# chymaera96/NeuralSampleID

Measured on AMD Instinct MI355X. Metric: audio clips/sec (contrastive step, grafp encoder), higher is better.
Workload: dtype bf16

## Files before the change

neuralsampleid_amd/build.py:

```python
import os
import subprocess
import sys
from concurrent.futures import ThreadPoolExecutor

PKG = os.path.dirname(os.path.abspath(__file__))
CSRC = os.path.join(PKG, "csrc")
ROOT = os.path.dirname(PKG)
LIB = os.path.join(PKG, "libnsid_hip.so")
OBJ_DIR = os.path.join(PKG, "csrc", "_obj")
SOURCES = ["tuning.hip", "gemm.hip", "gemm256.hip", "wsgemm.hip", "ffn_fused.hip", "ffn256_fused.hip", "mrconv_fused.hip", "wgrad.hip", "bn.hip", "knn.hip", "mr.hip", "ntxent.hip", "misc.hip"]
HIPCC = os.environ.get("HIPCC", "/opt/rocm/bin/hipcc")
FLAGS = ["-O3", "--offload-arch=gfx950", "-fPIC", "-std=c++17", "-Wall", "-Wno-unused-function",
         "-fno-gpu-rdc", "-I", os.path.join(ROOT, "include")]


def _newer(a, b):
    return not os.path.exists(b) or os.path.getmtime(a) > os.path.getmtime(b)


def _deps():
    hdrs = [os.path.join(CSRC, "nsid_common.h"), os.path.join(ROOT, "include", "nsid.h")]
    return max(os.path.getmtime(h) for h in hdrs)


def _check_flags() -> None:
    if "-DNSID_" in HIPCC or any(f.startswith("-DNSID_") for f in FLAGS):
        raise RuntimeError("refusing to build the product library with a -DNSID_* switch: use tools/build_variant.sh for diagnosis builds")


def _source_hash() -> str:
    import hashlib
    _check_flags()
    h = hashlib.sha256((HIPCC + " " + " ".join(f for f in FLAGS if f != os.path.join(ROOT, "include"))).encode())
    for f in [os.path.join(CSRC, s) for s in SOURCES] + [os.path.join(CSRC, "nsid_common.h"),
                                                         os.path.join(ROOT, "include", "nsid.h")]:
        h.update(open(f, "rb").read())
    return h.hexdigest()


def build_lib(force: bool = False, verbose: bool = True) -> str:
    stamp = LIB + ".srchash"
    digest = _source_hash()
    if not force and os.path.exists(LIB) and os.path.exists(stamp) and open(stamp).read().strip() == digest:
        return LIB
    force = True
    os.makedirs(OBJ_DIR, exist_ok=True)
    hdr_time = _deps()
    jobs = []
    for src in SOURCES:
        s = os.path.join(CSRC, src)
        o = os.path.join(OBJ_DIR, src.replace(".hip", ".o"))
        if force or _newer(s, o) or os.path.getmtime(o) < hdr_time:
            jobs.append((s, o))

    def compile_one(job):
        s, o = job
        cmd = [HIPCC, *FLAGS, "-c", s, "-o", o]
        r = subprocess.run(cmd, capture_output=True, text=True)
        if r.returncode != 0:
            raise RuntimeError(f"hipcc failed for {s}:\n{r.stderr}")
        if verbose and r.stderr.strip():
            print(r.stderr, file=sys.stderr)
        return o

    if jobs:
        with ThreadPoolExecutor(max_workers=min(6, len(jobs))) as ex:
            list(ex.map(compile_one, jobs))
    objs = [os.path.join(OBJ_DIR, s.replace(".hip", ".o")) for s in SOURCES]
    if jobs or not os.path.exists(LIB):
        r = subprocess.run([HIPCC, "--offload-arch=gfx950", "-shared", "-fPIC", "-o", LIB, *objs],
                           capture_output=True, text=True)
        if r.returncode != 0:
            raise RuntimeError("link failed:\n" + r.stderr)
        if verbose:
            print(f"built {LIB} ({os.path.getsize(LIB) / 1024:.0f} KB)")
    with open(stamp, "w") as f:
        f.write(digest)
    return LIB


if __name__ == "__main__":
    build_lib(force="--force" in sys.argv)
```

neuralsampleid_amd/csrc/gemm.hip:

```cpp
#include <algorithm>
#include <cstdlib>
#include "nsid_common.h"

namespace {

inline float act_slope(int act) { return act == NSID_ACT_RELU ? 0.f : (act == NSID_ACT_LEAKY ? 0.2f : 1.f); }

struct GemmArgs {
  const void* A; long lda; long a_goff;
  const void* B; long ldb; long b_goff;
  void* C; long ldc; long c_goff;
  int I, J, R;
  const float* a_scale; const float* a_shift; float a_slope; long a_aff_goff;
  const float* b_scale; const float* b_shift; float b_slope; long b_aff_goff;
  const float* bias; long bias_goff;
  const void* addend; long ldadd;
  float* stat; long stat_plane;
  long stat_ld;
  int rsplit;
  int rchunk;
  int atomic_out;
  int split_major;
  const void* bn_r; long bn_ldr;
  const float* bn_scale; const float* bn_shift; const float* bn_mean; const float* bn_invstd; float bn_slope;
// ... 934 lines not shown
  p.rchunk = (M + p.rsplit - 1) / p.rsplit;
  return launch_pad<64, 64, false, false, 2>(p, 1, static_cast<hipStream_t>(stream), act_dtype, false);
}

extern "C" int nsid_downsample3_bwd_data(const void* dout, const void* wp, const void* w_odd, int w_dtype, void* dx, int B,
                                         int N, int C, int Cout, int act_dtype, void* stream) {
  NSID_REQUIRE(dout && wp && w_odd && dx && B > 0 && N > 0 && N % 2 == 0 && C > 0 && Cout > 0 && NSID_DTYPE_OK(act_dtype));
  const int ch = act_dtype == NSID_BF16 ? 8 : 4;
  NSID_REQUIRE(C % ch == 0 && Cout % ch == 0 && nsid_aligned16(dout) && nsid_aligned16(wp) && nsid_aligned16(w_odd) &&
               nsid_aligned16(dx) && NSID_DTYPE_OK(w_dtype) && (w_dtype == NSID_F32 || act_dtype == NSID_BF16));
  const int No = N / 2, M = B * No;
  const long esz = act_dtype == NSID_BF16 ? 2 : 4, wsz = w_dtype == NSID_BF16 ? 2 : 4;
  hipStream_t s = static_cast<hipStream_t>(stream);
  const bool wb = w_dtype == NSID_BF16;
  GemmArgs p{};
  p.A = dout; p.lda = Cout; p.a_goff = Cout;
  p.B = static_cast<const char*>(wp) + (long)C * wsz; p.ldb = 3L * C; p.b_goff = 0;
  p.C = dx; p.ldc = 2L * C; p.c_goff = C;
  p.I = M; p.J = C; p.R = Cout;
  p.rsplit = 1; p.rchunk = Cout;
  p.bn_slope = 1.f;
  int rc = C <= 64 ? launch<128, 64, true, false>(p, 1, s, act_dtype, wb) : launch<128, 128, true, false>(p, 1, s, act_dtype, wb);
  if (rc != NSID_OK) return rc;
  GemmArgs q{};
  q.A = dout; q.lda = Cout; q.a_goff = 2L * Cout;
  q.B = w_odd; q.ldb = C; q.b_goff = 0;
  q.C = static_cast<char*>(dx) + (long)C * esz; q.ldc = 2L * C; q.c_goff = C;
  q.I = M; q.J = C; q.R = 2 * Cout;
  q.rsplit = 1; q.rchunk = 2 * Cout;
  q.bn_slope = 1.f;
  q.pad_period = No; q.pad_phase = No - 1; q.pad_c0 = Cout; q.pad_c1 = 2 * Cout; q.pad_safe = 0;
  return C <= 64 ? launch_pad<128, 64, true, false, 1>(q, 1, s, act_dtype, wb)
                 : launch_pad<128, 128, true, false, 1>(q, 1, s, act_dtype, wb);
}

void* g_gemm_trace_host = nullptr;
extern "C" int nsid_debug_gemm_trace(void* buf) {
  g_gemm_trace_host = buf;
  return hipMemcpyToSymbol(HIP_SYMBOL(g_gemm_trace), &buf, sizeof(buf)) == hipSuccess ? NSID_OK : NSID_EINVAL;
}
extern "C" int nsid_set_gemm_precision(int mode) {
  if (mode != NSID_GEMM_FP32 && mode != NSID_GEMM_BF16) return NSID_EINVAL;
  g_gemm_precision = mode;
  return NSID_OK;
}
extern "C" int nsid_get_gemm_precision(void) { return g_gemm_precision; }
extern "C" long nsid_gemm_g256_launches(void) { return g_g256_launches; }
extern "C" int nsid_row_tiles(int M) { return (M + NSID_ROW_TILE - 1) / NSID_ROW_TILE; }

static int linear_fwd_impl(const void* x, int ldx, const void* w, int w_dtype, const float* bias, void* out, int ldo,
                           int M, int Nout, int K, int groups, const float* in_scale, const float* in_shift, int act_in,
                           int act_out, float* stat, int ksplit, int act_dtype, const void* addend, int ldadd,
                           void* stream);

extern "C" int nsid_linear_fwd(const void* x, int ldx, const void* w, int w_dtype, const float* bias, void* out, int ldo,
                               int M, int Nout, int K, int groups, const float* in_scale, const float* in_shift,
                               int act_in, int act_out, float* stat, int ksplit, int act_dtype, void* stream) {
  return linear_fwd_impl(x, ldx, w, w_dtype, bias, out, ldo, M, Nout, K, groups, in_scale, in_shift, act_in, act_out, stat,
                         ksplit, act_dtype, nullptr, 0, stream);
}

extern "C" int nsid_linear_fwd_res(const void* x, int ldx, const void* w, int w_dtype, const float* bias,
                                   const void* addend, int ldadd, void* out, int ldo, int M, int Nout, int K, int groups,
                                   const float* in_scale, const float* in_shift, int act_in, int act_dtype,
                                   void* stream) {
  const int ch = act_dtype == NSID_BF16 ? 8 : 4;
  NSID_REQUIRE(addend && ldadd % ch == 0 && ldadd >= groups * Nout && nsid_aligned16(addend));
  return linear_fwd_impl(x, ldx, w, w_dtype, bias, out, ldo, M, Nout, K, groups, in_scale, in_shift, act_in,
                         NSID_ACT_NONE, nullptr, 1, act_dtype, addend, ldadd, stream);
}

static int linear_fwd_impl(const void* x, int ldx, const void* w, int w_dtype, const float* bias, void* out, int ldo,
                           int M, int Nout, int K, int groups, const float* in_scale, const float* in_shift, int act_in,
                           int act_out, float* stat, int ksplit, int act_dtype, const void* addend, int ldadd,
                           void* stream) {
  NSID_REQUIRE(x && w && out && M > 0 && Nout > 0 && K > 0 && groups > 0 && ksplit >= 1 && NSID_DTYPE_OK(act_dtype));
  NSID_REQUIRE(NSID_DTYPE_OK(w_dtype) && (w_dtype == NSID_F32 || (act_dtype == NSID_BF16 && K % 8 == 0)));
  const int ch = act_dtype == NSID_BF16 ? 8 : 4;
  NSID_REQUIRE(K % ch == 0 && ldx % ch == 0 && nsid_aligned16(x) && nsid_aligned16(w) && K % 4 == 0);
  NSID_REQUIRE(act_dtype == NSID_F32 || (ksplit == 1 && (act_out == NSID_ACT_NONE || act_out == NSID_ACT_RELU) && Nout % 8 == 0 && ldo % 8 == 0));
  NSID_REQUIRE(act_out != NSID_ACT_RELU || (ksplit == 1 && stat == nullptr && addend == nullptr));
  NSID_REQUIRE((ldx >= groups * K || (groups == 1 && ldx > 0)) && ldo >= groups * Nout);
  NSID_REQUIRE(Nout % 4 == 0 && ldo % 4 == 0 && nsid_aligned16(out) && (bias == nullptr || nsid_aligned16(bias)));
  NSID_REQUIRE((in_scale == nullptr) == (in_shift == nullptr));
  NSID_REQUIRE(ksplit == 1 || (stat == nullptr && (act_out == NSID_ACT_NONE || (act_out == NSID_ACT_ELU && act_dtype == NSID_F32))));
  NSID_REQUIRE(act_in != NSID_ACT_ELU && (act_out == NSID_ACT_NONE || act_out == NSID_ACT_ELU || act_out == NSID_ACT_RELU));
  NSID_REQUIRE(in_scale != nullptr || act_in == NSID_ACT_NONE ||
               (act_in == NSID_ACT_RELU && act_dtype == NSID_BF16 && w_dtype == NSID_BF16));
  GemmArgs p{};
  p.A = x; p.lda = ldx; p.a_goff = K;
  p.B = w; p.ldb = K; p.b_goff = (long)Nout * K;
  p.C = out; p.ldc = ldo; p.c_goff = Nout;
  p.I = M; p.J = Nout; p.R = K;
  p.a_scale = in_scale; p.a_shift = in_shift; p.a_slope = act_slope(act_in); p.a_aff_goff = K;
  p.bias = bias; p.bias_goff = Nout;
  p.addend = addend; p.ldadd = ldadd;
  p.stat = stat; p.stat_ld = (long)groups * Nout; p.stat_plane = (long)nsid_row_tiles(M) * groups * Nout;
  p.rsplit = ksplit;
  p.rchunk = (K + ksplit - 1) / ksplit;
  p.atomic_out = ksplit > 1;
  p.relu_out = act_out == NSID_ACT_RELU;
  hipStream_t s = static_cast<hipStream_t>(stream);
  const long t128 = (long)nsid_row_tiles(M) * ((Nout + 127) / 128) * groups;
  const bool half = g_gemm_precision == NSID_GEMM_BF16 || act_dtype == NSID_BF16;
  const int force_narrow = (int)nsid_tune(NSID_T_fwd_narrow);
  bool narrow = half ? (Nout <= 64 || (Nout <= 128 && K <= 256 && in_scale == nullptr)) : Nout <= 64;
  if (half && t128 < 128) narrow = true;
  if (force_narrow >= 0 && Nout > 64) narrow = force_narrow != 0;
  const bool wb = w_dtype == NSID_BF16;
  if ((nsid_tune(NSID_T_ws_gemm) & 1) && act_dtype == NSID_BF16 && wb && ksplit == 1 && act_out == NSID_ACT_NONE && addend == nullptr &&
      act_in != NSID_ACT_ELU) {
    const int rcw = nsid_ws_fwd_launch(x, ldx, w, bias, out, ldo, M, Nout, K, groups, in_scale, in_shift, act_slope(act_in), stat,
                                       p.stat_plane, p.stat_ld, s);
    if (rcw != 1) { nsid_count(NSID_C_ws_fwd); return rcw; }
  }
  const long g256_min = nsid_tune(NSID_T_g256_min);
  if (g256_min > 0 && (stat == nullptr || nsid_tune(NSID_T_g256_train) != 0) && act_dtype == NSID_BF16 && wb && groups == 1 && in_scale == nullptr && ksplit == 1 &&
      (act_out == NSID_ACT_NONE || act_out == NSID_ACT_RELU) && act_in == NSID_ACT_NONE && ldx >= K &&
      (long)(M / 256) * (Nout / 256) >= g256_min) {
    const int rc256 = nsid_gemm256_fwd_launch(x, ldx, w, bias, addend, ldadd, out, ldo, M, Nout, K, act_out == NSID_ACT_RELU, stat,
                                              p.stat_plane, p.stat_ld, s);
    if (rc256 != 1) { ++g_g256_launches; nsid_count(NSID_C_gemm256); return rc256; }
  }
  const int rc = narrow ? launch<128, 64, true, true>(p, groups, s, act_dtype, wb) : launch<128, 128, true, true>(p, groups, s, act_dtype, wb);
  if (rc != NSID_OK || act_out != NSID_ACT_ELU) return rc;
  const long n = (long)M * groups * Nout;
  NSID_LAUNCH(elu_inplace_kernel, dim3((int)((n + 255) / 256 > 2048 ? 2048 : (n + 255) / 256)), dim3(256), 0, s,
              static_cast<float*>(out), (long)M, groups * Nout, (long)ldo);
  return nsid_launch_status();
}

struct AbnArgs {
  const void* r; const float* coef4; int act; void* dr;
};
static int linear_bwd_data_impl(const void* dout, int ldd, const void* w, int w_dtype, const void* addend, int ldadd,
                                void* din, int ldi, int M, int Nout, int K, int groups, int act_dtype, void* stream,
                                const void* bn_r, const float* bn_scale, const float* bn_shift, const float* bn_mean,
                                const float* bn_invstd, int bn_act, float* bn_partial, const AbnArgs* abn = nullptr);

extern "C" int nsid_linear_bwd_data(const void* dout, int ldd, const void* w, int w_dtype, const void* addend, int ldadd,
                                    void* din, int ldi, int M, int Nout, int K, int groups, int act_dtype,
                                    void* stream) {
  return linear_bwd_data_impl(dout, ldd, w, w_dtype, addend, ldadd, din, ldi, M, Nout, K, groups, act_dtype, stream,
                              nullptr, nullptr, nullptr, nullptr, nullptr, NSID_ACT_NONE, nullptr);
}

extern "C" int nsid_linear_bwd_data_bn(const void* dout, int ldd, const void* w, int w_dtype, const void* addend,
                                       int ldadd, void* din, int ldi, int M, int Nout, int K, int groups, int act_dtype,
                                       const void* bn_r, const float* bn_scale, const float* bn_shift,
                                       const float* bn_mean, const float* bn_invstd, int bn_act, float* bn_partial,
                                       void* stream) {
  NSID_REQUIRE(bn_r && bn_scale && bn_shift && bn_mean && bn_invstd && bn_partial && act_dtype == NSID_BF16);
  NSID_REQUIRE(ldi == groups * K && (groups * K) % 8 == 0 && nsid_aligned16(bn_r));
  NSID_REQUIRE(bn_act == NSID_ACT_NONE || bn_act == NSID_ACT_RELU || bn_act == NSID_ACT_LEAKY);
  return linear_bwd_data_impl(dout, ldd, w, w_dtype, addend, ldadd, din, ldi, M, Nout, K, groups, act_dtype, stream,
                              bn_r, bn_scale, bn_shift, bn_mean, bn_invstd, bn_act, bn_partial);
}

extern "C" int nsid_linear_bwd_data_bnapply(const void* dy, const void* r, const float* coef4, int act, void* dr, const void* w,
                                            int w_dtype, const void* addend, int ldadd, void* din, int ldi, int M, int Nout, int K,
                                            int groups, int act_dtype, const void* bn_r, const float* bn_scale,
                                            const float* bn_shift, const float* bn_mean, const float* bn_invstd, int bn_act,
                                            float* bn_partial, void* stream) {
  NSID_REQUIRE(dy && r && coef4 && dr && nsid_aligned16(r) && nsid_aligned16(dr) && nsid_aligned16(coef4));
  NSID_REQUIRE(dr != dy && dr != r);
  NSID_REQUIRE(act == NSID_ACT_NONE || act == NSID_ACT_RELU || act == NSID_ACT_LEAKY);
  if (act_dtype != NSID_BF16 || w_dtype != NSID_BF16 || (groups * Nout) % 8 != 0) return 1;
  if (bn_r != nullptr) {
    NSID_REQUIRE(bn_scale && bn_shift && bn_mean && bn_invstd && bn_partial && ldi == groups * K && (groups * K) % 8 == 0 &&
                 nsid_aligned16(bn_r));
    NSID_REQUIRE(bn_act == NSID_ACT_NONE || bn_act == NSID_ACT_RELU || bn_act == NSID_ACT_LEAKY);
  }
  const AbnArgs abn{r, coef4, act, dr};
  return linear_bwd_data_impl(dy, groups * Nout, w, w_dtype, addend, ldadd, din, ldi, M, Nout, K, groups, act_dtype, stream, bn_r,
                              bn_scale, bn_shift, bn_mean, bn_invstd, bn_act, bn_partial, &abn);
}

static int linear_bwd_data_impl(const void* dout, int ldd, const void* w, int w_dtype, const void* addend, int ldadd,
                                void* din, int ldi, int M, int Nout, int K, int groups, int act_dtype, void* stream,
                                const void* bn_r, const float* bn_scale, const float* bn_shift, const float* bn_mean,
                                const float* bn_invstd, int bn_act, float* bn_partial, const AbnArgs* abn) {
  NSID_REQUIRE(dout && w && din && M > 0 && Nout > 0 && K > 0 && groups > 0 && NSID_DTYPE_OK(act_dtype));
  NSID_REQUIRE(NSID_DTYPE_OK(w_dtype) && (w_dtype == NSID_F32 || (act_dtype == NSID_BF16 && K % 8 == 0)));
  const bool wb = w_dtype == NSID_BF16;
  const int ch = act_dtype == NSID_BF16 ? 8 : 4;
  NSID_REQUIRE(Nout % ch == 0 && K % ch == 0 && ldd % ch == 0 && ldi % ch == 0 && nsid_aligned16(dout) && nsid_aligned16(w));
  NSID_REQUIRE(addend == nullptr || ldadd % ch == 0);
  NSID_REQUIRE(ldd >= groups * Nout && ldi >= groups * K && ldi % 4 == 0 && nsid_aligned16(din));
  NSID_REQUIRE(addend == nullptr || (ldadd % 4 == 0 && ldadd >= groups * K && nsid_aligned16(addend)));
  GemmArgs p{};
  p.A = dout; p.lda = ldd; p.a_goff = Nout;
  p.B = w; p.ldb = K; p.b_goff = (long)Nout * K;
  p.C = din; p.ldc = ldi; p.c_goff = K;
  p.I = M; p.J = K; p.R = Nout;
  p.addend = addend; p.ldadd = ldadd;
  p.rsplit = 1; p.rchunk = Nout;
  p.bn_r = bn_r; p.bn_ldr = (long)groups * K;
  p.bn_scale = bn_scale; p.bn_shift = bn_shift; p.bn_mean = bn_mean; p.bn_invstd = bn_invstd;
  p.bn_slope = act_slope(bn_act);
  p.bn_partial = bn_partial; p.bn_ld = (long)groups * K; p.bn_plane = (long)nsid_row_tiles(M) * groups * K;
  hipStream_t s = static_cast<hipStream_t>(stream);
  const long t128 = (long)nsid_row_tiles(M) * ((K + 127) / 128) * groups;
  const bool half = g_gemm_precision == NSID_GEMM_BF16 || act_dtype == NSID_BF16;
  const int force_narrow = (int)nsid_tune(NSID_T_bwd_narrow);
  bool narrow = half ? (K <= 64 || (K <= 128 && Nout <= 256)) : K <= 64;
  if (half && t128 < 128) narrow = true;
  if (force_narrow >= 0 && K > 64) narrow = force_narrow != 0;
  if ((nsid_tune(NSID_T_ws_gemm) & (abn ? 4 : 2)) && act_dtype == NSID_BF16 && wb &&
      (bn_r == nullptr || bn_partial != nullptr)) {
    const int rcw = nsid_ws_bwd_data_launch(dout, ldd, w, addend, ldadd, din, ldi, M, Nout, K, groups, bn_r, p.bn_ldr, bn_scale, bn_shift,
                                            bn_mean, bn_invstd, p.bn_slope, bn_partial, p.bn_plane, p.bn_ld, abn ? abn->r : nullptr,
                                            abn ? abn->coef4 : nullptr, (long)groups * Nout, abn ? act_slope(abn->act) : 1.f,
                                            abn ? abn->dr : nullptr, (long)groups * Nout, s);
    if (rcw != 1) { nsid_count(abn ? NSID_C_ws_bwd_bnapply : NSID_C_ws_bwd_data); return rcw; }
  }
  if (abn != nullptr) {
    narrow = K <= 64;
    p.abn_r = abn->r; p.abn_coef = abn->coef4; p.abn_plane = (long)groups * Nout; p.abn_slope = act_slope(abn->act);
    p.abn_dr = abn->dr; p.abn_lddr = (long)groups * Nout;
    if (K % (narrow ? 64 : 128) != 0 || M % 128 != 0 || Nout % 64 != 0) return 1;
  }
  if (act_dtype == NSID_F32 && addend == nullptr && bn_r == nullptr && abn == nullptr && groups == 1 && Nout >= 1024 && ldi == K) {
    const long tiles = (long)nsid_row_tiles(M) * ((K + (narrow ? 63 : 127)) / (narrow ? 64 : 128));
    const long maxt = nsid_tune(NSID_T_bwd_split_max_tiles);
    const long S = maxt > 0 && tiles <= maxt ? std::min<long>(256 / tiles, Nout / 256) : 1;
    if (S > 1) {
      const int rcz = nsid_fill_zero(din, (size_t)M * K * 4, stream);
      if (rcz != NSID_OK) return rcz;
      p.rsplit = (int)S;
      p.rchunk = (int)((Nout + S - 1) / S);
      p.atomic_out = 1;
      nsid_count(NSID_C_gemm_bwd_split);
    }
  }
  if (narrow) return launch<128, 64, true, false>(p, groups, s, act_dtype, wb);
  return launch<128, 128, true, false>(p, groups, s, act_dtype, wb);
}

extern "C" int nsid_linear_bwd_weight(const void* dout, int ldd, const void* x, int ldx, float* dw, int M, int Nout,
                                      int K, int groups, const float* in_scale, const float* in_shift, int act_in,
                                      int act_dtype, void* stream) {
  NSID_REQUIRE(dout && x && dw && M > 0 && Nout > 0 && K > 0 && groups > 0 && NSID_DTYPE_OK(act_dtype));
  const int ch = act_dtype == NSID_BF16 ? 8 : 4;
  NSID_REQUIRE(Nout % ch == 0 && K % ch == 0 && ldd % ch == 0 && ldx % ch == 0 && nsid_aligned16(dout) && nsid_aligned16(x));
  NSID_REQUIRE((in_scale == nullptr) == (in_shift == nullptr));
  GemmArgs p{};
  p.A = dout; p.lda = ldd; p.a_goff = Nout;
  p.B = x; p.ldb = ldx; p.b_goff = K;
  p.C = dw; p.ldc = K; p.c_goff = (long)Nout * K;
  p.I = Nout; p.J = K; p.R = M;
  p.b_scale = in_scale; p.b_shift = in_shift; p.b_slope = act_slope(act_in); p.b_aff_goff = K;
  p.atomic_out = 1;
  const bool use_wide = nsid_tune(NSID_T_wgrad_wide) != 0;
  if (use_wide && act_dtype == NSID_BF16 && nsid_aligned16(dout) && nsid_aligned16(x) &&
      (in_scale == nullptr || (nsid_aligned16(in_scale) && nsid_aligned16(in_shift)))) {
    const int rc = nsid_wgrad2_launch(dout, ldd, x, ldx, dw, M, Nout, K, groups, in_scale, in_shift, act_slope(act_in),
                                      static_cast<hipStream_t>(stream));
    if (rc != 1) return rc;
  }
  const long rect = nsid_tune(NSID_T_wgrad_rect);
  const long wg_rect = nsid_tune(NSID_T_wgrad_wgs_rect);
  const long wg_sq = nsid_tune(NSID_T_wgrad_wgs_sq);
  if (rect && act_dtype == NSID_BF16 && Nout % 128 == 0 && K % 64 == 0 && M % 1024 == 0) {
    const long tiles_r = (long)(Nout / 128) * (K / 64) * groups;
    const long S = std::min<long>(M / 1024, std::max<long>(1, wg_rect / tiles_r));
    const long rect_min = nsid_tune(NSID_T_wgrad_rect_min);
    if (tiles_r * S >= rect_min) {
      p.rsplit = (int)S;
      p.rchunk = (int)(M / S);
      return launch<128, 64, false, false>(p, groups, static_cast<hipStream_t>(stream), act_dtype);
    }
  }
  const bool half = g_gemm_precision == NSID_GEMM_BF16 || act_dtype == NSID_BF16;
  const long t128 = (long)((Nout + 127) / 128) * ((K + 127) / 128) * groups;
  const bool small = half || (Nout <= 64 || K <= 64) || t128 * ((M + 511) / 512) < 256;
  const int bm = small ? 64 : 128;
  const long tiles = (long)((Nout + bm - 1) / bm) * ((K + bm - 1) / bm) * groups;
  long S;
  if (half) {
    S = std::min<long>((M + 1023) / 1024, std::max<long>(1, wg_sq / tiles));
    const long sq_min = nsid_tune(NSID_T_wgrad_sq_min);
    S = std::max<long>(S, (sq_min + tiles - 1) / tiles);
    S = std::min<long>(S, (M + 255) / 256);
  } else {
    S = std::min<long>((512 + tiles - 1) / tiles, (M + 511) / 512);
  }
  int rsplit = (int)std::max<long>(S, 1);
  p.rsplit = rsplit;
  p.rchunk = (M + rsplit - 1) / rsplit;
  hipStream_t s = static_cast<hipStream_t>(stream);
  if (small) return launch<64, 64, false, false>(p, groups, s, act_dtype);
  return launch<128, 128, false, false>(p, groups, s, act_dtype);
}

extern "C" int nsid_linear_bwd_weight_grouped(const nsid_wgrad_problem* problems, int n, int act_dtype, int max_workgroups,
                                              void* stream) {
  NSID_REQUIRE(problems && n > 0 && NSID_DTYPE_OK(act_dtype) && max_workgroups >= 0);
  const bool st16 = act_dtype == NSID_BF16;
  const int ch = st16 ? 8 : 4;
  hipStream_t s = static_cast<hipStream_t>(stream);
  const long rows_target = std::max<long>(128, nsid_tune(NSID_T_wgg_rows));
  const long rows_sq = std::max<long>(128, nsid_tune(NSID_T_wgg_rows_sq)), rows_gen = std::max<long>(32, nsid_tune(NSID_T_wgg_rows_gen));
  const bool use_w3 = nsid_tune(NSID_T_wgg_w3) != 0;
  constexpr int NCLS = 7;
  WgGroupArgs ga[NCLS];
  long wgs[NCLS] = {0, 0, 0, 0, 0, 0, 0};
  const bool half = g_gemm_precision == NSID_GEMM_BF16 || st16;
  for (int c = 0; c < NCLS; ++c) ga[c].n = 0;
  auto flush = [&](int c) -> int {
    if (ga[c].n == 0) return NSID_OK;
    ga[c].wg0[ga[c].n] = (int)wgs[c];
    long gsz = wgs[c];
    if (max_workgroups > 0 && gsz > max_workgroups) gsz = std::max(8, max_workgroups / 8 * 8);
    const dim3 grid((unsigned)gsz), block(256);
    if (c == 3 || c == 4) {
      nsid_count(NSID_C_wgrad_grouped);
      nsid_count(NSID_C_wgrad_grouped_w3);
      const int rc3 = nsid_wgrad3_grouped_launch(ga[c], (int)gsz, c == 4, s);
      ga[c].n = 0;
      wgs[c] = 0;
      return rc3;
    }
    if (c == 0) NSID_LAUNCH((wgrad_grouped_kernel<128, 64, true>), grid, block, 0, s, ga[c]);
    else if (c == 1) NSID_LAUNCH((wgrad_grouped_kernel<64, 64, true>), grid, block, 0, s, ga[c]);
    else if (c == 2) NSID_LAUNCH((wgrad_grouped_kernel<64, 64, false>), grid, block, 0, s, ga[c]);
    else if (c == 5) NSID_LAUNCH((wgrad_grouped_kernel<64, 64, false, true, true, 2>), grid, block, 0, s, ga[c]);
    else if (half) NSID_LAUNCH((wgrad_grouped_kernel<64, 64, false, true, false>), grid, block, 0, s, ga[c]);
    else NSID_LAUNCH((wgrad_grouped_kernel<64, 64, false, false, false>), grid, block, 0, s, ga[c]);
    nsid_count(NSID_C_wgrad_grouped);
    ga[c].n = 0;
    wgs[c] = 0;
    return nsid_launch_status();
  };
  for (int i = 0; i < n; ++i) {
    const nsid_wgrad_problem& q = problems[i];
    const int nseg = q.dout[1] != nullptr ? 2 : 1;
    NSID_REQUIRE(q.dout[0] && q.x[0] && q.dw && q.M > 0 && q.Nout > 0 && q.K > 0 && q.groups > 0);
    NSID_REQUIRE((q.dout[1] == nullptr) == (q.x[1] == nullptr));
    NSID_REQUIRE(q.Nout % ch == 0 && q.K % ch == 0 && q.ldd % ch == 0 && q.ldx % ch == 0 && q.ds_out_nodes >= 0);
    const bool ds = q.ds_out_nodes > 0;
    NSID_REQUIRE(!ds || (st16 && q.groups == 1 && q.K % 3 == 0 && (q.K / 3) % 8 == 0 && q.M % q.ds_out_nodes == 0 && q.in_scale[0] == nullptr &&
                         q.ldx == q.K / 3));
    for (int v = 0; v < nseg; ++v) {
      NSID_REQUIRE(nsid_aligned16(q.dout[v]) && nsid_aligned16(q.x[v]));
      NSID_REQUIRE((q.in_scale[v] == nullptr) == (q.in_shift[v] == nullptr));
      NSID_REQUIRE((q.in_scale[v] == nullptr) == (q.in_scale[0] == nullptr));
      NSID_REQUIRE(q.in_scale[v] == nullptr || (nsid_aligned16(q.in_scale[v]) && nsid_aligned16(q.in_shift[v])));
    }
    const bool rows_ok = q.M % 128 == 0;
    int cls = (rows_ok && q.Nout % 128 == 0 && q.K % 64 == 0) ? 0 : ((rows_ok && q.Nout % 64 == 0 && q.K % 64 == 0) ? 1 : 2);
    if (cls == 0 && use_w3 && q.K % 128 == 0) cls = q.in_scale[0] != nullptr ? 4 : 3;
    if (ds) cls = 5;
    if (!st16) cls = 6;
    const int bm = (cls == 0 || cls == 3 || cls == 4) ? 128 : 64, bn = (cls == 3 || cls == 4) ? 128 : 64;
    const long rows_cls = (cls == 1 || cls == 5) ? rows_sq : ((cls == 2 || cls == 6) ? rows_gen : rows_target);
    WgProb w{};
    for (int v = 0; v < 2; ++v) {
      w.A[v] = q.dout[v]; w.B[v] = q.x[v]; w.bsc[v] = q.in_scale[v]; w.bsh[v] = q.in_shift[v];
    }
    w.C = q.dw; w.lda = q.ldd; w.ldb = q.ldx; w.I = q.Nout; w.J = q.K; w.R = q.M; w.groups = q.groups;
    if (ds) {
      const int C = q.K / 3;
      for (int v = 0; v < nseg; ++v) w.B[v] = static_cast<const char*>(q.x[v]) - (long)C * 2;
      w.ldb = 2 * C; w.pad_period = q.ds_out_nodes; w.pad_c1 = C;
    }
    w.slope = act_slope(q.act_in);
    long S = 1;
    if (cls != 2 && cls != 5 && cls != 6) {
      while (q.M % (2 * S) == 0 && (q.M / (2 * S)) % 128 == 0 && q.M / (2 * S) >= rows_cls) S *= 2;
      w.rchunk = (int)(q.M / S);
    } else {
      S = std::max<long>(1, (q.M + rows_cls - 1) / rows_cls);
      w.rchunk = (int)(((q.M + S - 1) / S + 31) / 32 * 32);
      S = (q.M + w.rchunk - 1) / w.rchunk;
    }
    w.seg_splits = (int)S;
    w.nsplit = (int)S * nseg;
    w.tiles = ((q.Nout + bm - 1) / bm) * ((q.K + bn - 1) / bn);
    const long tg = (long)w.tiles * q.groups;
    long nwg = tg * w.nsplit;
    if (w.nsplit < 8 && 8 % w.nsplit == 0) nwg = (tg + 8 / w.nsplit - 1) / (8 / w.nsplit) * 8;
    w.nwg = (int)nwg;
    NSID_REQUIRE(nwg < (1L << 30));
    if (ga[cls].n == WGG_MAXP || wgs[cls] + nwg > (1L << 30)) {
      const int rc = flush(cls);
      if (rc != NSID_OK) return rc;
    }
    ga[cls].wg0[ga[cls].n] = (int)wgs[cls];
    ga[cls].prob[ga[cls].n++] = w;
    wgs[cls] += (nwg + 7) / 8 * 8;
  }
  for (int c = 0; c < NCLS; ++c) {
    const int rc = flush(c);
    if (rc != NSID_OK) return rc;
  }
  return NSID_OK;
}
```

neuralsampleid_amd/csrc/nsid_common.h:

```cpp
#pragma once
#include <hip/hip_runtime.h>
#include <stdint.h>
#include <stdio.h>

#include "../../include/nsid.h"

typedef float f32x2 __attribute__((ext_vector_type(2)));
typedef float f32x4 __attribute__((ext_vector_type(4)));
typedef uint32_t u32x4 __attribute__((ext_vector_type(4)));
typedef __bf16 bf16x4 __attribute__((ext_vector_type(4)));
typedef __bf16 bf16x8 __attribute__((ext_vector_type(8)));

template <typename T> struct Chunk;
template <> struct Chunk<float> {
  static constexpr int N = 4;
  __device__ static __forceinline__ void load(const float* p, float* v) {
    const f32x4 x = *reinterpret_cast<const f32x4*>(p);
#pragma unroll
    for (int e = 0; e < 4; ++e) v[e] = x[e];
  }
  __device__ static __forceinline__ void store(float* p, const float* v) {
    *reinterpret_cast<f32x4*>(p) = f32x4{v[0], v[1], v[2], v[3]};
  }
};
template <> struct Chunk<__bf16> {
  static constexpr int N = 8;
  __device__ static __forceinline__ void load(const __bf16* p, float* v) {
    const bf16x8 x = *reinterpret_cast<const bf16x8*>(p);
#pragma unroll
    for (int e = 0; e < 8; ++e) v[e] = (float)x[e];
  }
  __device__ static __forceinline__ void store(__bf16* p, const float* v) {
    bf16x8 x;
#pragma unroll
    for (int e = 0; e < 8; ++e) x[e] = (__bf16)v[e];
    *reinterpret_cast<bf16x8*>(p) = x;
  }
};

template <int N>
__device__ __forceinline__ void load_channels(const float* __restrict__ p, int c, float* v) {
#pragma unroll
  for (int e = 0; e < N; e += 4) {
    const f32x4 x = *reinterpret_cast<const f32x4*>(p + c + e);
    v[e] = x[0]; v[e + 1] = x[1]; v[e + 2] = x[2]; v[e + 3] = x[3];
  }
}

#define NSID_DISPATCH_DTYPE(dtype, T, ...)                    \
  do {                                                        \
    if ((dtype) == NSID_BF16) { typedef __bf16 T; __VA_ARGS__; } \
    else { typedef float T; __VA_ARGS__; }                    \
  } while (0)
#define NSID_DTYPE_OK(d) ((d) == NSID_F32 || (d) == NSID_BF16)

#define NSID_WAVE 64

__device__ __forceinline__ float nsid_act(float v, int act) {
  switch (act) {
    case NSID_ACT_RELU: return v < 0.f ? 0.f : v;
    case NSID_ACT_LEAKY: return v > 0.f ? v : 0.2f * v;
    case NSID_ACT_ELU: return v > 0.f ? v : expm1f(v);
    default: return v;
  }
}
__device__ __forceinline__ float nsid_act_grad(float pre, int act) {
  switch (act) {
    case NSID_ACT_RELU: return pre > 0.f ? 1.f : 0.f;
    case NSID_ACT_LEAKY: return pre > 0.f ? 1.f : 0.2f;
    default: return 1.f;
  }
}

__device__ __forceinline__ float wave_sum(float v) {
  v += __builtin_bit_cast(float, __builtin_amdgcn_update_dpp(0, __builtin_bit_cast(int, v), 0xB1, 0xF, 0xF, true));
  v += __builtin_bit_cast(float, __builtin_amdgcn_update_dpp(0, __builtin_bit_cast(int, v), 0x4E, 0xF, 0xF, true));
  v += __builtin_bit_cast(float, __builtin_amdgcn_update_dpp(0, __builtin_bit_cast(int, v), 0x141, 0xF, 0xF, true));
  v += __builtin_bit_cast(float, __builtin_amdgcn_update_dpp(0, __builtin_bit_cast(int, v), 0x140, 0xF, 0xF, true));
  v += __builtin_bit_cast(float, __builtin_amdgcn_update_dpp(0, __builtin_bit_cast(int, v), 0x142, 0xA, 0xF, true));
  v += __builtin_bit_cast(float, __builtin_amdgcn_update_dpp(0, __builtin_bit_cast(int, v), 0x143, 0xC, 0xF, true));
  return __builtin_bit_cast(float, __builtin_amdgcn_readlane(__builtin_bit_cast(int, v), 63));
}
__device__ __forceinline__ double wave_sum_d(double v) {
#pragma unroll
  for (int o = 32; o > 0; o >>= 1) v += __shfl_xor(v, o, 64);
  return v;
}
__device__ __forceinline__ float wave_max(float v) {
#pragma unroll
  for (int o = 32; o > 0; o >>= 1) v = fmaxf(v, __shfl_xor(v, o, 64));
  return v;
}
__device__ __forceinline__ float wave_min(float v) {
#pragma unroll
  for (int o = 32; o > 0; o >>= 1) v = fminf(v, __shfl_xor(v, o, 64));
  return v;
}

#define NSID_LAUNCH(kernel, grid, block, shmem, stream, ...)                \
  do {                                                                      \
    (void)hipGetLastError();                                                \
    hipLaunchKernelGGL(kernel, grid, block, shmem, stream, __VA_ARGS__);    \
  } while (0)

static inline int nsid_launch_status() {
  hipError_t e = hipGetLastError();
  if (e != hipSuccess) fprintf(stderr, "[nsid] kernel launch failed: %s\n", hipGetErrorString(e));
  return e == hipSuccess ? NSID_OK : NSID_ELAUNCH;
}
static inline bool nsid_aligned16(const void* p) { return (reinterpret_cast<uintptr_t>(p) & 15u) == 0; }

#define NSID_REQUIRE(cond) \
  do {                     \
    if (!(cond)) return NSID_EINVAL; \
  } while (0)

#define NSID_TUNING_TABLE(X)                                                                                                  \
  X(stream_max_wg, 2048)                              \
  X(bn_bwd_apply_max_wg, 384)        \
  X(gemm_deep_ks, 2)                 \
  X(gemm_deep_pd, 2)                                        \
  X(gemm_deep_max_wg, 1024)     \
  X(gemm_deep_ec, 0)                    \
  X(gemm_deep_kinds, 5)         \
  X(bwd_split_max_tiles, 64)    \
  X(fwd_narrow, -1)                                         \
  X(bwd_narrow, -1)                                                                                                           \
  X(g256_min, 512)                                  \
  X(g256_train, 0)                            \
  X(g256_grid, 0)                                           \
  X(wgrad_wide, 1)                                     \
  X(wgrad_rect, 1)                                                                          \
  X(wgrad_wgs_rect, 256)                         \
  X(wgrad_wgs_sq, 1024)                                                                                                       \
  X(wgrad_rect_min, 256)                                                                                                      \
  X(wgrad_sq_min, 256)                                                                                                        \
  X(w3_wgs, 256)                                                                                                              \
  X(w3_min_tiles, 64)                                                                                                         \
  X(knn_strips, 0)                                            \
  X(knn_pair_min, 512)                 \
  X(knn_raw16, 1)               \
  X(knn_raw_wpe, 6)             \
  X(knn_sel_min_n, 128)               \
  X(mr_grid_stride, 0)                              \
  X(mr_split, 0)                                             \
  X(ffn_regs, 3)                \
  X(mr_key_min_k, 8)            \
  X(mr_bwd_sorted_min_k, 3)     \
  X(ffn_waves, 8)                                                \
  X(ffn256, 1)                  \
  X(mrconv_variant, 7)          \
  X(mrconv_pg_wgs, 768)         \
  X(wgg_rows, 4096)             \
  X(wgg_rows_sq, 1024)          \
  X(wgg_rows_gen, 512)          \
  X(bn_fin_tiles, 0)            \
  X(wgg_w3, 1)                  \
  X(ws_gemm, 7)

enum NsidTuneKey {
#define NSID_TUNE_ENUM(name, def) NSID_T_##name,
  NSID_TUNING_TABLE(NSID_TUNE_ENUM)
#undef NSID_TUNE_ENUM
  NSID_T_COUNT
};
extern long g_nsid_tune[NSID_T_COUNT];
static inline long nsid_tune(NsidTuneKey k) { return g_nsid_tune[k]; }

#define NSID_COUNTER_TABLE(X)                                                                  \
  X(gemm_fwd) X(gemm_bwd_data) X(gemm_bwd_weight)              \
  X(gemm_full)                                    \
  X(gemm_ks2)                                                           \
  X(gemm_pd4) X(gemm_ec)                                                \
  X(gemm_bwd_split)          \
  X(gemm_split_major)           \
  X(gemm_affine_load)          \
  X(gemm_relu_load)                                                                             \
  X(gemm_bn_sums)              \
  X(gemm_bn_apply_load)     \
  X(gemm256)                                                                   \
  X(ws_fwd) X(ws_bwd_data) X(ws_bwd_bnapply)                    \
  X(wgrad_rect) X(wgrad_square) X(wgrad3) X(wgrad_grouped) X(wgrad_grouped_w3)                                                       \
  X(bn_bwd_apply) X(bn_bwd_apply_capped)                                                        \
  X(knn2) X(knn2_pair) X(knn2_raw) X(knn_rank) X(knn_sel) X(knn_strips) X(knn_big)                                                  \
  X(mr_fwd_lds) X(mr_fwd_grid) X(mr_fwd_key) X(mr_bwd_sorted)                                                                  \
  X(ffn_fused)                                 \
  X(mrconv_fused)

enum NsidCounterKey {
#define NSID_CNT_ENUM(name) NSID_C_##name,
  NSID_COUNTER_TABLE(NSID_CNT_ENUM)
#undef NSID_CNT_ENUM
  NSID_C_COUNT
};
extern long g_nsid_counter[NSID_C_COUNT];
static inline void nsid_count(NsidCounterKey k) { ++g_nsid_counter[k]; }

constexpr int WGG_MAXP = 28;
struct WgProb {
  const void* A[2];
  const void* B[2];
  const float* bsc[2];
  const float* bsh[2];
  float* C;
  int lda, ldb, I, J, R;
  int groups, rchunk;
  int seg_splits, nsplit;
  int tiles, nwg;
  float slope;
  int pad_period, pad_c1;
};
struct WgGroupArgs {
  int n, pad;
  int wg0[WGG_MAXP + 1];
  WgProb prob[WGG_MAXP];
};
static_assert(sizeof(WgProb) == 128 && sizeof(WgGroupArgs) + 256 <= 4096, "the problem table travels in the kernel arguments");


__device__ __forceinline__ bool wgg_decode(const WgGroupArgs& ga, const int w, int& pi, int& split, int& bid, int& g, int& seg) {
  pi = 0;
  for (int i = 1; i < ga.n; ++i) pi += (w >= ga.wg0[i]) ? 1 : 0;
  pi = __builtin_amdgcn_readfirstlane(pi);
  const WgProb& q = ga.prob[pi];
  const int l = w - ga.wg0[pi];
  if (l >= q.nwg) return false;
  const int S = q.nsplit;
  int rest;
  if (S < 8 && (8 % S) == 0) {
    const int x = l & 7, per = 8 / S;
    split = x % S;
    rest = (l >> 3) * per + x / S;
  } else {
    split = l % S;
    rest = l / S;
  }
  if (rest >= q.tiles * q.groups) return false;
  g = rest / q.tiles;
  bid = rest % q.tiles;
  seg = split >= q.seg_splits ? 1 : 0;
  split -= seg * q.seg_splits;
  return true;
}
int nsid_wgrad3_grouped_launch(const WgGroupArgs& ga, int grid, bool affine, hipStream_t stream);

int nsid_wgrad2_launch(const void* dout, int ldd, const void* x, int ldx, float* dw, int M, int Nout, int K, int groups,
                       const float* in_scale, const float* in_shift, float slope, hipStream_t stream);

int nsid_gemm256_fwd_launch(const void* x, int ldx, const void* w, const float* bias, const void* addend, int ldadd, void* out,
                            int ldo, int M, int Nout, int K, bool relu_out, float* stat, long stat_plane, long stat_ld,
                            hipStream_t stream);
int nsid_ws_fwd_launch(const void* x, int ldx, const void* w, const float* bias, void* out, int ldo, int M, int Nout, int K,
                       int groups, const float* in_scale, const float* in_shift, float in_slope, float* stat, long stat_plane,
                       long stat_ld, hipStream_t stream);
int nsid_ws_bwd_data_launch(const void* dout, int ldd, const void* w, const void* addend, int ldadd, void* din, int ldi, int M, int Nout,
                            int K, int groups, const void* bn_r, long bn_ldr, const float* bn_scale, const float* bn_shift,
                            const float* bn_mean, const float* bn_invstd, float bn_slope, float* bn_partial, long bn_plane, long bn_ld,
                            const void* abn_r, const float* abn_coef, long abn_plane, float abn_slope, void* abn_dr, long abn_lddr,
                            hipStream_t stream);
int nsid_ffn256_fused_launch(const void* x, const void* w1, const float* b1, const void* w2, const float* b2, void* out, int M, int C,
                             int H, hipStream_t stream);
extern void* g_gemm_trace_host;
```

Measured before the change: 35530.

## Add 256x256-tile grouped weight-gradient kernel with async LDS ring pipeline

```diff
diff --git a/neuralsampleid_amd/build.py b/neuralsampleid_amd/build.py
--- a/neuralsampleid_amd/build.py
+++ b/neuralsampleid_amd/build.py
@@ -8,7 +8,7 @@
 ROOT = os.path.dirname(PKG)
 LIB = os.path.join(PKG, "libnsid_hip.so")
 OBJ_DIR = os.path.join(PKG, "csrc", "_obj")
-SOURCES = ["tuning.hip", "gemm.hip", "gemm256.hip", "wsgemm.hip", "ffn_fused.hip", "ffn256_fused.hip", "mrconv_fused.hip", "wgrad.hip", "bn.hip", "knn.hip", "mr.hip", "ntxent.hip", "misc.hip"]
+SOURCES = ["tuning.hip", "gemm.hip", "gemm256.hip", "wsgemm.hip", "ffn_fused.hip", "ffn256_fused.hip", "mrconv_fused.hip", "wgrad.hip", "wgrad256.hip", "bn.hip", "knn.hip", "mr.hip", "ntxent.hip", "misc.hip"]
 HIPCC = os.environ.get("HIPCC", "/opt/rocm/bin/hipcc")
 FLAGS = ["-O3", "--offload-arch=gfx950", "-fPIC", "-std=c++17", "-Wall", "-Wno-unused-function",
          "-fno-gpu-rdc", "-I", os.path.join(ROOT, "include")]
diff --git a/neuralsampleid_amd/csrc/gemm.hip b/neuralsampleid_amd/csrc/gemm.hip
--- a/neuralsampleid_amd/csrc/gemm.hip
+++ b/neuralsampleid_amd/csrc/gemm.hip
@@ -1260,9 +1260,11 @@
   const long rows_target = std::max<long>(128, nsid_tune(NSID_T_wgg_rows));
   const long rows_sq = std::max<long>(128, nsid_tune(NSID_T_wgg_rows_sq)), rows_gen = std::max<long>(32, nsid_tune(NSID_T_wgg_rows_gen));
   const bool use_w3 = nsid_tune(NSID_T_wgg_w3) != 0;
-  constexpr int NCLS = 7;
+  const bool use_w4 = nsid_tune(NSID_T_wgrad256) != 0;
+  const long rows_w4 = std::max<long>(128, nsid_tune(NSID_T_wgg_rows256));
+  constexpr int NCLS = 8;
   WgGroupArgs ga[NCLS];
-  long wgs[NCLS] = {0, 0, 0, 0, 0, 0, 0};
+  long wgs[NCLS] = {0, 0, 0, 0, 0, 0, 0, 0};
   const bool half = g_gemm_precision == NSID_GEMM_BF16 || st16;
   for (int c = 0; c < NCLS; ++c) ga[c].n = 0;
   auto flush = [&](int c) -> int {
@@ -1278,6 +1280,14 @@
       ga[c].n = 0;
       wgs[c] = 0;
       return rc3;
+    }
+    if (c == 7) {
+      nsid_count(NSID_C_wgrad_grouped);
+      nsid_count(NSID_C_wgrad_grouped_256);
+      const int rc4 = nsid_wgrad4_grouped_launch(ga[c], (int)gsz, s);
+      ga[c].n = 0;
+      wgs[c] = 0;
+      return rc4;
     }
     if (c == 0) NSID_LAUNCH((wgrad_grouped_kernel<128, 64, true>), grid, block, 0, s, ga[c]);
     else if (c == 1) NSID_LAUNCH((wgrad_grouped_kernel<64, 64, true>), grid, block, 0, s, ga[c]);
@@ -1308,10 +1318,14 @@
     const bool rows_ok = q.M % 128 == 0;
     int cls = (rows_ok && q.Nout % 128 == 0 && q.K % 64 == 0) ? 0 : ((rows_ok && q.Nout % 64 == 0 && q.K % 64 == 0) ? 1 : 2);
     if (cls == 0 && use_w3 && q.K % 128 == 0) cls = q.in_scale[0] != nullptr ? 4 : 3;
+    if (cls == 0 || cls == 3 || cls == 4) {
+      if (use_w4 && q.Nout % 256 == 0 && q.K % 256 == 0) cls = 7;
+    }
     if (ds) cls = 5;
     if (!st16) cls = 6;
-    const int bm = (cls == 0 || cls == 3 || cls == 4) ? 128 : 64, bn = (cls == 3 || cls == 4) ? 128 : 64;
-    const long rows_cls = (cls == 1 || cls == 5) ? rows_sq : ((cls == 2 || cls == 6) ? rows_gen : rows_target);
+    const bool w4 = cls == 7;
+    const int bm = w4 ? 256 : ((cls == 0 || cls == 3 || cls == 4) ? 128 : 64), bn = w4 ? 256 : ((cls == 3 || cls == 4) ? 128 : 64);
+    const long rows_cls = (cls == 1 || cls == 5) ? rows_sq : ((cls == 2 || cls == 6) ? rows_gen : (w4 ? rows_w4 : rows_target));
     WgProb w{};
     for (int v = 0; v < 2; ++v) {
       w.A[v] = q.dout[v]; w.B[v] = q.x[v]; w.bsc[v] = q.in_scale[v]; w.bsh[v] = q.in_shift[v];
diff --git a/neuralsampleid_amd/csrc/nsid_common.h b/neuralsampleid_amd/csrc/nsid_common.h
--- a/neuralsampleid_amd/csrc/nsid_common.h
+++ b/neuralsampleid_amd/csrc/nsid_common.h
@@ -156,6 +156,8 @@
   X(wgg_rows_gen, 512)          \
   X(bn_fin_tiles, 0)            \
   X(wgg_w3, 1)                  \
+  X(wgrad256, 1)                \
+  X(wgg_rows256, 4096)          \
   X(ws_gemm, 7)
 
 enum NsidTuneKey {
@@ -180,7 +182,7 @@
   X(gemm_bn_apply_load)     \
   X(gemm256)                                                                   \
   X(ws_fwd) X(ws_bwd_data) X(ws_bwd_bnapply)                    \
-  X(wgrad_rect) X(wgrad_square) X(wgrad3) X(wgrad_grouped) X(wgrad_grouped_w3)                                                       \
+  X(wgrad_rect) X(wgrad_square) X(wgrad3) X(wgrad_grouped) X(wgrad_grouped_w3) X(wgrad_grouped_256)                                                 \
   X(bn_bwd_apply) X(bn_bwd_apply_capped)                                                        \
   X(knn2) X(knn2_pair) X(knn2_raw) X(knn_rank) X(knn_sel) X(knn_strips) X(knn_big)                                                  \
   X(mr_fwd_lds) X(mr_fwd_grid) X(mr_fwd_key) X(mr_bwd_sorted)                                                                  \
@@ -243,6 +245,7 @@
   return true;
 }
 int nsid_wgrad3_grouped_launch(const WgGroupArgs& ga, int grid, bool affine, hipStream_t stream);
+int nsid_wgrad4_grouped_launch(const WgGroupArgs& ga, int grid, hipStream_t stream);
 
 int nsid_wgrad2_launch(const void* dout, int ldd, const void* x, int ldx, float* dw, int M, int Nout, int K, int groups,
                        const float* in_scale, const float* in_shift, float slope, hipStream_t stream);
diff --git a/neuralsampleid_amd/csrc/wgrad256.hip b/neuralsampleid_amd/csrc/wgrad256.hip
--- /dev/null
+++ b/neuralsampleid_amd/csrc/wgrad256.hip
@@ -0,0 +1,168 @@
+#include <cstdlib>
+#include "nsid_common.h"
+
+namespace {
+
+constexpr int W4_T = 256, W4_BK = 32, W4_THREADS = 512;
+constexpr int W4_ROW = W4_T * 2;
+constexpr int W4_OP = W4_BK * W4_ROW;
+constexpr int W4_SLOT = 2 * W4_OP;
+constexpr int W4_RING = 4 * W4_SLOT;
+static_assert(W4_RING <= 160 * 1024, "one workgroup per CU");
+
+typedef __attribute__((address_space(3))) void* w4_lds_ptr;
+
+template <int N>
+__device__ __forceinline__ void w4_wait_vm() {
+  static_assert(N >= 0 && N < 64, "6-bit counter");
+  __builtin_amdgcn_s_waitcnt((N & 0xF) | ((N >> 4) << 14) | (7 << 4) | (0xF << 8));
+}
+__device__ __forceinline__ void w4_wait_lgkm0() { __builtin_amdgcn_s_waitcnt(0xC07F); }
+
+__device__ __forceinline__ void w4_glds16(const char* sbase, unsigned voff, unsigned dst) {
+  unsigned keep;
+  asm volatile("s_mov_b32 %0, m0\n\ts_mov_b32 m0, %3\n\ts_nop 0\n\tglobal_load_lds_dwordx4 %1, %2\n\ts_mov_b32 m0, %0"
+               : "=&s"(keep) : "v"(voff), "s"(sbase), "s"(dst) : "memory");
+}
+
+__device__ __forceinline__ bf16x8 w4_frag(const char* p) {
+  typedef bf16x4 __attribute__((address_space(3))) * lds_bf16x4_ptr;
+  const bf16x4 t0 = __builtin_amdgcn_ds_read_tr16_b64_v4bf16((lds_bf16x4_ptr)(p));
+  const bf16x4 t1 = __builtin_amdgcn_ds_read_tr16_b64_v4bf16((lds_bf16x4_ptr)(p + 4 * W4_ROW));
+  return __builtin_shufflevector(t0, t1, 0, 1, 2, 3, 4, 5, 6, 7);
+}
+
+template <bool BAFF>
+__device__ __forceinline__ void wgrad4_item(const WgProb& q, const int split, const int tile, const int g, const int seg, char* lds) {
+  const int tid = threadIdx.x, lane = tid & 63;
+  const int wave = __builtin_amdgcn_readfirstlane(tid >> 6);
+  const int wr = wave >> 2, wc = wave & 3;
+  const int lr = lane & 15, rq = lane >> 4;
+  const int tiles_j = q.J / W4_T;
+  const int i0 = (tile / tiles_j) * W4_T, j0 = (tile % tiles_j) * W4_T;
+  const int rbeg = split * q.rchunk;
+  const int nst = q.rchunk / W4_BK;
+
+  const bool stage_x = wave >= 4;
+  const long ld2 = (long)(stage_x ? q.ldb : q.lda) * 2;
+  const int h = lane >> 5, sw = wave & 3;
+  unsigned voff[2];
+#pragma unroll
+  for (int par = 0; par < 2; ++par) {
+    const int f = (2 * par + h) | ((sw & 1) << 2);
+    voff[par] = (unsigned)(h * ld2) + ((unsigned)((lane & 31) * 16) ^ (unsigned)(f << 5));
+  }
+  const char* gbase = stage_x ? static_cast<const char*>(q.B[seg]) + ((long)g * q.J + j0) * 2
+                              : static_cast<const char*>(q.A[seg]) + ((long)g * q.I + i0) * 2;
+  gbase += (long)(rbeg + 8 * sw) * ld2;
+  const unsigned lds0 = (unsigned)(size_t)(w4_lds_ptr)lds + (stage_x ? W4_OP : 0) + sw * 8 * W4_ROW;
+  auto issue = [&](int st, int slot) {
+    const char* s = gbase + (long)st * W4_BK * ld2;
+#pragma unroll
+    for (int i = 0; i < 4; ++i) w4_glds16(s + 2 * i * ld2, voff[i & 1], lds0 + slot * W4_SLOT + 2 * i * W4_ROW);
+  };
+
+  const int fr = lr >> 2, fsw = fr | ((rq & 1) << 2);
+  const int fbase = (8 * rq + fr) * W4_ROW + 8 * (lr & 3);
+  int aoff[8], boff[4];
+#pragma unroll
+  for (int a = 0; a < 8; ++a) aoff[a] = fbase + (((wr * 8 + a) ^ fsw) << 5);
+#pragma unroll
+  for (int b = 0; b < 4; ++b) boff[b] = W4_OP + fbase + (((wc * 4 + b) ^ fsw) << 5);
+
+  float bsc[4], bsh[4];
+  if (BAFF) {
+#pragma unroll
+    for (int b = 0; b < 4; ++b) {
+      const long jj = (long)g * q.J + j0 + 64 * wc + 16 * b + lr;
+      bsc[b] = q.bsc[seg][jj];
+      bsh[b] = q.bsh[seg][jj];
+    }
+  }
+  const float slope = q.slope;
+
+  f32x4 acc[8][4];
+#pragma unroll
+  for (int a = 0; a < 8; ++a)
+#pragma unroll
+    for (int b = 0; b < 4; ++b) acc[a][b] = f32x4{0.f, 0.f, 0.f, 0.f};
+
+  auto compute = [&](int slot) {
+    const char* st = lds + slot * W4_SLOT;
+    bf16x8 fa[8], fb[4];
+#pragma unroll
+    for (int b = 0; b < 4; ++b) fb[b] = w4_frag(st + boff[b]);
+#pragma unroll
+    for (int a = 0; a < 8; ++a) fa[a] = w4_frag(st + aoff[a]);
+    if (BAFF) {
+#pragma unroll
+      for (int b = 0; b < 4; ++b) {
+        bf16x8 o;
+#pragma unroll
+        for (int e = 0; e < 8; e += 2) {
+          const f32x2 v = f32x2{bsc[b], bsc[b]} * f32x2{(float)fb[b][e], (float)fb[b][e + 1]} + f32x2{bsh[b], bsh[b]};
+          const f32x2 w = v * slope;
+          o[e] = (__bf16)fmaxf(v[0], w[0]);
+          o[e + 1] = (__bf16)fmaxf(v[1], w[1]);
+        }
+        fb[b] = o;
+      }
+    }
+#pragma unroll
+    for (int a = 0; a < 8; ++a)
+#pragma unroll
+      for (int b = 0; b < 4; ++b) acc[a][b] = __builtin_amdgcn_mfma_f32_16x16x32_bf16(fa[a], fb[b], acc[a][b], 0, 0, 0);
+  };
+
+  const int last = nst - 1;
+  issue(0, 0);
+  issue(min(1, last), 1);
+  issue(min(2, last), 2);
+#define NSID_W4_STEP(U)                                        \
+  do {                                                         \
+    w4_wait_vm<8>();                                           \
+    w4_wait_lgkm0();                                           \
+    __builtin_amdgcn_s_barrier();                              \
+    __builtin_amdgcn_sched_barrier(0);                         \
+    issue(min(st + (U) + 3, last), ((U) + 3) & 3);             \
+    compute(U);                                                \
+    __builtin_amdgcn_sched_barrier(0);                         \
+  } while (0)
+  for (int st = 0; st < nst; st += 4) {
+    NSID_W4_STEP(0);
+    NSID_W4_STEP(1);
+    NSID_W4_STEP(2);
+    NSID_W4_STEP(3);
+  }
+#undef NSID_W4_STEP
+  w4_wait_vm<0>();
+
+  float* C = q.C + (long)g * q.I * q.J;
+#pragma unroll
+  for (int a = 0; a < 8; ++a)
+#pragma unroll
+    for (int b = 0; b < 4; ++b)
+#pragma unroll
+      for (int r = 0; r < 4; ++r)
+        atomicAdd(C + (long)(i0 + 128 * wr + 16 * a + 4 * rq + r) * q.J + (j0 + 64 * wc + 16 * b + lr), acc[a][b][r]);
+}
+
+__global__ __launch_bounds__(W4_THREADS, 2) void wgrad4_grouped_kernel(const WgGroupArgs ga) {
+  __shared__ __attribute__((aligned(1024))) char lds[W4_RING];
+  const int total = ga.wg0[ga.n];
+  for (int w = blockIdx.x; w < total; w += gridDim.x) {
+    int pi, split, bid, g, seg;
+    if (wgg_decode(ga, w, pi, split, bid, g, seg)) {
+      const WgProb& q = ga.prob[pi];
+      if (q.bsc[seg] != nullptr) wgrad4_item<true>(q, split, bid, g, seg, lds);
+      else wgrad4_item<false>(q, split, bid, g, seg, lds);
+    }
+  }
+}
+
+}
+
+int nsid_wgrad4_grouped_launch(const WgGroupArgs& ga, int grid, hipStream_t stream) {
+  NSID_LAUNCH(wgrad4_grouped_kernel, dim3(grid), dim3(W4_THREADS), 0, stream, ga);
+  return nsid_launch_status();
+}
```

New measurement: 36070, median of 6. +1.5%, better.
